# mlcolab/Pathfinder.jl

Measured on AMD Instinct MI355X. Metric: ELBO draws/sec (multipathfinder hot path: fit + ELBO + pool + PSIS + resample), higher is better.
Workload: dtype f64

## Files before the change

### pathfinder.jl_amd/csrc/elbo_kernels.hip

```cpp
#include "pfmi_common.h"
#include "elbo_args.h"
#include "logpdf_lane.h"
#include <stdlib.h>

#define ELBO_THREADS 256


template <int TGT, int RPAD>
struct TargetAcc {
    double q = 0.0, tau = 0.0;
    double tr[RPAD > 0 ? RPAD : 1];
    __device__ __forceinline__ void init() {
#pragma unroll
        for (int j = 0; j < (RPAD > 0 ? RPAD : 1); ++j) tr[j] = 0.0;
    }
    __device__ __forceinline__ void row(const ElboArgs &A, int i, double x) {
        if (TGT == 1) {
            const double e = x - A.t_mean[i];
            q += A.t_a[i] * e * e;
            if (RPAD > 0) {
                const double *wr = A.t_wd + (size_t)i * RPAD;
#pragma unroll
                for (int j = 0; j < RPAD; ++j) tr[j] += wr[j] * e;
            }
        } else if (TGT == 2) {
            if (i == 0) tau = x; else q += x * x;
        }
    }
    __device__ __forceinline__ double finish(const ElboArgs &A) {
        if (TGT == 1) {
            double corr = 0.0;
            if (RPAD > 0) {
#pragma unroll
                for (int j = 0; j < RPAD; ++j) {
                    double g = 0.0;
#pragma unroll
                    for (int l = 0; l <= j; ++l) g += A.t_g[j * RPAD + l] * tr[l];
                    corr += g * g;
// ... 121 lines not shown
#pragma unroll
                for (int j = 0; j < KPAD; ++j) v -= row[j] * tv[j];
                const double xi = mu[i] + sqa[i] * v;
                tg.row(A, i, xi);
                if (X) X[i] = xi;
            }
        }
    }
    *out_lq = ((double)d * PF_LOG2PI + A.logdet[p] + usq) / -2.0;
    *out_lp = tg.finish(A);
}

__global__ __launch_bounds__(256) void pf_elbo_reduce_kernel(int64_t N, const int64_t *__restrict__ off,
                                                             const int32_t *__restrict__ path_of,
                                                             const int32_t *__restrict__ status,
                                                             const double *__restrict__ logp,
                                                             const double *__restrict__ logq,
                                                             double *__restrict__ elbo, double *__restrict__ se,
                                                             int64_t vcap, int seg_len, const int32_t *__restrict__ npts) {
    int p = blockIdx.x;
    const int tid = threadIdx.x;
    if (seg_len > 0) {
        const int k = blockIdx.x / seg_len, l = blockIdx.x - k * seg_len;
        if (l >= npts[k]) return;
        p = (int)((int64_t)k * vcap + l);
    }
    __shared__ double red[8];
    const bool first = ((int64_t)p == off[path_of[p]]);
    if (first || status[p] != PFMI_FIT_OK || N <= 0) {
        if (tid == 0) { elbo[p] = NAN; se[p] = NAN; }
        return;
    }
    const double *lp = logp + (size_t)p * N, *lq = logq + (size_t)p * N;
    double s = 0.0;
    for (int64_t n = tid; n < N; n += 256) s += lp[n] - lq[n];
    s = pf_block_sum1(s, red);
    const double mean = s / (double)N;
    double v = 0.0;
    for (int64_t n = tid; n < N; n += 256) { const double r = (lp[n] - lq[n]) - mean; v += r * r; }
    v = pf_block_sum1(v, red);
    if (tid == 0) {
        elbo[p] = mean;
        se[p] = sqrt((v / (double)(N - 1)) / (double)N);
    }
}

__global__ __launch_bounds__(64) void pf_elbo_argmax_kernel(int K, const int64_t *__restrict__ off, const int32_t *__restrict__ npts,
                                                           const double *__restrict__ elbo, int64_t *__restrict__ best_iter) {
    const int k = blockIdx.x, lane = threadIdx.x;
    if (k >= K) return;
    const int64_t p0 = off[k];
    const int L = npts ? npts[k] - 1 : (int)(off[k + 1] - p0 - 1);
    if (L <= 0) { if (lane == 0) best_iter[k] = 0; return; }
    double xmax = 0.0;
    int imax = 0x7FFFFFFF, have = 0;
    for (int l = 1 + lane; l <= L; l += 64) {
        const double xi = elbo[p0 + l];
        if (isnan(xi)) continue;
        if (!have || xi > xmax) { xmax = xi; imax = l; have = 1; }
    }
#pragma unroll
    for (int o = 32; o >= 1; o >>= 1) {
        const double xo = __shfl_xor(xmax, o, 64);
        const int io = __shfl_xor(imax, o, 64), ho = __shfl_xor(have, o, 64);
        const bool take = ho && (!have || xo > xmax || (xo == xmax && io < imax));
        if (take) { xmax = xo; imax = io; have = 1; }
    }
    if (lane == 0) best_iter[k] = have ? imax : 1;
}

__global__ void pf_logratio_kernel(int64_t n, const double *__restrict__ lp, const double *__restrict__ lq,
                                   double *__restrict__ lr) {
// ... 206 lines not shown
```

### pathfinder.jl_amd/csrc/pfmi_common.h

```cpp
#pragma once
#include <hip/hip_runtime.h>
#include <stdint.h>
#include <chrono>
#include <functional>
#include <memory>
#include <string>
#include <map>
#include <set>
#include <type_traits>
#include <vector>

#include "../../include/pfmi.h"
#include "pfmi_icdftab.h"

#define PF_LOG2PI 1.8378770664093454835606594728112352797227949472755668

void pf_set_error(const char *fmt, ...);
#define PF_HIP(call)                                                                              \
    do {                                                                                          \
        hipError_t e__ = (call);                                                                  \
        if (e__ != hipSuccess) {                                                                  \
            pf_set_error("%s failed: %s (%s:%d)", #call, hipGetErrorString(e__), __FILE__, __LINE__); \
            return PFMI_ERR_HIP;                                                                  \
        }                                                                                         \
// ... 186 lines not shown
    int64_t N_e = 0;
    DevBuf seeds;
    DevBuf logp, logq;
    DevBuf elbo, se;
    DevBuf best_iter;
    DevBuf fit_list;
    DevBuf ubuf;
    DevBuf xbuf;
    DevBuf scratch;
    DevBuf mix;
    DevBuf qf_share_s[2];
    uint32_t qf_epoch_s[2] = {0, 0};
    int qf_slot = 0;
    bool qf_no_share = false;
    int64_t qf_lost_total = 0;
    std::map<std::string, int64_t> qf_plans;
    std::map<std::string, int64_t> draw_plans;
    std::map<std::string, int64_t> fit_plans;

    bool pooled = false;
    int64_t N_r = 0;
    DevBuf pool;
    DevBuf pool_lr;
    DevBuf pool_lp, pool_lq;
    DevBuf pool_points;
    DevBuf pool_seeds;
    int64_t S_w = 0;
    DevBuf lw;
    DevBuf w;
    DevBuf psis_out;
    DevBuf psis_aux;
    DevBuf tailbuf;
    DevBuf cdf;
    DevBuf idx;
    DevBuf gbuf;
    DevBuf sortk, sorti;
    DevBuf cb_x[2], cb_lp[2];
    void *pin_x[2] = {nullptr, nullptr}, *pin_lp[2] = {nullptr, nullptr};
    size_t pin_x_cap = 0, pin_lp_cap = 0;
    hipEvent_t cb_ev[2] = {nullptr, nullptr};
#define PF_DCB_NB 2
    DevBuf dcb_x[PF_DCB_NB], dcb_lp[PF_DCB_NB];
    hipStream_t s_cb[PF_DCB_NB - 1] = {};
    hipEvent_t sg_cb[PF_DCB_NB] = {};
    double cb_seconds = 0.0;
    double cb_bytes_d2h = 0.0;
    double cb_bytes_dev = 0.0;
    bool opt_pending = false;
    LbcState lbc;
    DevBuf lc_X, lc_out, lc_x, lc_g, lc_p, lc_gram, lc_st, lc_ctr;
    int64_t *lc_status = nullptr;
    int32_t opt_K = 0, opt_cap = 0;
    HmcState hmc;
    DevBuf hm_X, hm_out, hm_x0, hm_x, hm_wg, hm_wt, hm_v, hm_st, hm_pts, hm_seeds, hm_eps;
    DevBuf hm_draws, hm_lp, hm_acc, hm_de, hm_div;
    DevBuf hm_pX, hm_pout, hm_pv;
    DevBuf hm_adapt;
    DevBuf hm_scale;
    DevBuf hm_chees;
    DevBuf hm_metric;
    std::vector<double> scale_staged;
    int32_t scale_staged_K = 0;
    DevBuf nt_vec, nt_st, nt_depth, nt_nleap, nt_pev, nt_ctr;
    int64_t *nt_status = nullptr;
    std::map<std::string, int64_t> hmc_plans;
    DevBuf cd_ws, cd_in;
// ... 533 lines not shown
```

### pathfinder.jl_amd/csrc/psis_kernels.hip

```cpp
#include "pfmi_common.h"
#include <stdlib.h>
#include <stddef.h>

#define PSIS_THREADS 1024
#ifndef PSIS_PROF
#define PSIS_PROF 0
#endif
#if PSIS_PROF
#define PS_STAMP(k) do { if (threadIdx.x == 0) { const long long t_ = wall_clock64(); ps_t[k] = t_ - ps_last; ps_last = t_; } } while (0)
#else
#define PS_STAMP(k) do { } while (0)
#endif
#define TAILCAP 4096

#define PF_KEY_NAN 0xFFF8000000000000ull
__device__ __forceinline__ uint64_t pf_key_of(double x) {
    uint64_t b = (uint64_t)__double_as_longlong(x);
    const uint64_t k = (b >> 63) ? ~b : (b | 0x8000000000000000ull);
    return (x != x) ? PF_KEY_NAN : k;
}
__device__ __forceinline__ double pf_val_of(uint64_t k) {
    uint64_t b = (k >> 63) ? (k & 0x7FFFFFFFFFFFFFFFull) : ~k;
    return __longlong_as_double((long long)b);
}
// ... 103 lines not shown
    const unsigned long long ti = st->prefix;
    int npow = 1;
    while (npow < R) npow <<= 1;
    for (int t = tid; t < npow; t += nt) { tkeys[t] = ~0ull; tidx[t] = 0xFFFFFFFFu; }
    if (tid == 0) st->count = 0u;
    __syncthreads();
    pf_foreach_batched(vals, S, [&](long long i, double x) {
        const uint64_t k = pf_key_of(x);
        if (k > tk || (k == tk && (unsigned long long)i >= ti)) {
            const unsigned slot = atomicAdd(&st->count, 1u);
            if (slot < (unsigned)TAILCAP) { tkeys[slot] = k; tidx[slot] = (uint32_t)i; }
        }
    });
    __syncthreads();
    for (int size = 2; size <= npow; size <<= 1) {
        for (int stride = size >> 1; stride > 0; stride >>= 1) {
            for (int t = tid; t < npow / 2; t += nt) {
                const int lo = 2 * t - (t & (stride - 1));
                const int hi = lo + stride;
                const bool up = ((lo & size) == 0);
                const uint64_t ka = tkeys[lo], kb = tkeys[hi];
                const uint32_t ia = tidx[lo], ib = tidx[hi];
                const bool a_gt_b = (ka > kb) || (ka == kb && ia > ib);
                if (a_gt_b == up) { tkeys[lo] = kb; tkeys[hi] = ka; tidx[lo] = ib; tidx[hi] = ia; }
            }
            __syncthreads();
        }
    }
}

#define PSIS_MULTI_MIN 8192
#define PSIS_MW 64
#define PSIS_MT 256
struct PsisAux {
    unsigned long long kmax, kmin_inv;
    unsigned hist[4096];
    unsigned cand_count, done, replaced, ti0;
    unsigned long long tk0;
    double mx, se_tail, pareto_k, sigma;
    int M, pad;
    double partial[PSIS_MW];
    unsigned long long cand_key[TAILCAP];
    unsigned cand_idx[TAILCAP];
    double tail_val[TAILCAP];
    unsigned tail_idx[TAILCAP];
};
__device__ __forceinline__ int pf_psis_shift0(unsigned long long kmin, unsigned long long kmax) {
    const unsigned long long diff = kmin ^ kmax;
    const int top = diff ? 63 - __clzll((long long)diff) : 0;
    return top >= 11 ? top - 11 : 0;
}
__global__ __launch_bounds__(PSIS_MT) void pf_psis_minmax_kernel(long long S, const double *__restrict__ lr, PsisAux *aux) {
    unsigned long long kmax = 0ull, kinv = 0ull;
    for (long long i = (long long)blockIdx.x * PSIS_MT + threadIdx.x; i < S; i += (long long)PSIS_MW * PSIS_MT) {
        const unsigned long long k = pf_key_of(lr[i]);
        kmax = k > kmax ? k : kmax; kinv = ~k > kinv ? ~k : kinv;
    }
    for (int off = 32; off > 0; off >>= 1) {
        const unsigned long long a = __shfl_xor(kmax, off, 64), b = __shfl_xor(kinv, off, 64);
        kmax = a > kmax ? a : kmax; kinv = b > kinv ? b : kinv;
    }
    if ((threadIdx.x & 63) == 0) { atomicMax(&aux->kmax, kmax); atomicMax(&aux->kmin_inv, kinv); }
}
__global__ __launch_bounds__(PSIS_MT) void pf_psis_hist_kernel(long long S, const double *__restrict__ lr, PsisAux *aux) {
    __shared__ unsigned h[4096];
    for (int b = threadIdx.x; b < 4096; b += PSIS_MT) h[b] = 0u;
    __syncthreads();
    const int sh = pf_psis_shift0(~aux->kmin_inv, aux->kmax);
    for (long long i = (long long)blockIdx.x * PSIS_MT + threadIdx.x; i < S; i += (long long)PSIS_MW * PSIS_MT)
        atomicAdd(&h[(unsigned)((pf_key_of(lr[i]) >> sh) & 0xFFFull)], 1u);
    __syncthreads();
    for (int b = threadIdx.x; b < 4096; b += PSIS_MT) if (h[b]) atomicAdd(&aux->hist[b], h[b]);
}
__global__ __launch_bounds__(PSIS_MT) void pf_psis_compact_kernel(long long S, const double *__restrict__ lr, PsisAux *aux, int R) {
    __shared__ unsigned part[PSIS_MT];
    __shared__ int s_bin, s_ok;
    const int tid = threadIdx.x;
    unsigned loc[16], sum = 0u;
#pragma unroll
// ... 9 lines not shown
            if (cum < (unsigned)R && cum + loc[j] >= (unsigned)R) { s_bin = 4095 - 16 * tid - j; s_ok = (cum + loc[j] <= (unsigned)TAILCAP); break; }
            cum += loc[j];
        }
    }
    __syncthreads();
    const int bin = s_bin;
    if (blockIdx.x == 0 && tid == 0) aux->done = (bin >= 0 && s_ok) ? 1u : 0u;
    if (bin < 0 || !s_ok) return;
    const int sh = pf_psis_shift0(~aux->kmin_inv, aux->kmax);
    for (long long i = (long long)blockIdx.x * PSIS_MT + tid; i < S; i += (long long)PSIS_MW * PSIS_MT) {
        const unsigned long long k = pf_key_of(lr[i]);
        if ((int)((k >> sh) & 0xFFFull) >= bin) {
            const unsigned slot = atomicAdd(&aux->cand_count, 1u);
            if (slot < (unsigned)TAILCAP) { aux->cand_key[slot] = k; aux->cand_idx[slot] = (unsigned)i; }
        }
    }
}
__device__ __forceinline__ bool pf_psis_is_tail(const PsisAux *aux, long long i, double x) {
    const unsigned long long k = pf_key_of(x);
    return aux->replaced && (k > aux->tk0 || (k == aux->tk0 && (unsigned long long)i > (unsigned long long)aux->ti0));
}
__global__ __launch_bounds__(PSIS_MT) void pf_psis_sum_kernel(long long S, const double *__restrict__ lr, PsisAux *aux) {
    __shared__ double red[PSIS_MT / 64];
    const double mx = aux->mx;
    double se = 0.0;
    if (isfinite(mx))
        for (long long i = (long long)blockIdx.x * PSIS_MT + threadIdx.x; i < S; i += (long long)PSIS_MW * PSIS_MT) {
            const double x = lr[i];
            if (!pf_psis_is_tail(aux, i, x)) se += exp(x - mx);
        }
    se = pf_block_sum1(se, red);
    if (threadIdx.x == 0) aux->partial[blockIdx.x] = se;
}
__global__ __launch_bounds__(PSIS_MT) void pf_psis_norm_kernel(long long S, const double *__restrict__ lr, const PsisAux *aux,
                                                              double *__restrict__ lw, double *__restrict__ wout,
                                                              double *__restrict__ out, const double *__restrict__ tail_val,
                                                              const unsigned *__restrict__ tail_idx) {
    if (tail_val == nullptr) { tail_val = aux->tail_val; tail_idx = aux->tail_idx; }
    const double mx = aux->mx;
    double se = aux->se_tail;
    for (int b = 0; b < PSIS_MW; ++b) se += aux->partial[b];
    const double lse = isfinite(mx) ? mx + log(se) : mx;
    for (long long i = (long long)blockIdx.x * PSIS_MT + threadIdx.x; i < S; i += (long long)PSIS_MW * PSIS_MT) {
        const double x = lr[i];
        if (!pf_psis_is_tail(aux, i, x)) { const double v = x - lse; lw[i] = v; wout[i] = exp(v); }
    }
    if (blockIdx.x == 0) {
        if (aux->replaced)
            for (int t = threadIdx.x; t < aux->M; t += PSIS_MT) {
                const double v = tail_val[t] - lse;
                lw[tail_idx[t]] = v; wout[tail_idx[t]] = exp(v);
            }
        if (threadIdx.x == 0) { out[0] = aux->pareto_k; out[1] = (double)aux->M; out[2] = aux->sigma; out[3] = lse; }
    }
}

template <bool MULTI>
__device__ __forceinline__ void pf_psis_segment(long long S, const double *__restrict__ lr, double *__restrict__ lw,
                                                double *__restrict__ wout, double *__restrict__ out, int M, PsisAux *aux) {
    const int tid = threadIdx.x, nt = blockDim.x, lane = tid & 63, wave = tid >> 6, nw = nt >> 6;
    __shared__ uint64_t tkeys[TAILCAP];
    __shared__ uint32_t tidx[TAILCAP];
    __shared__ SelectState st;
    __shared__ double red[PSIS_THREADS / 64];
    __shared__ double s_theta[128], s_ll[128];
    __shared__ double s_sigma, s_mu;

#if PSIS_PROF
    long long ps_t[8] = {0, 0, 0, 0, 0, 0, 0, 0}, ps_last = wall_clock64();
#endif
    double pareto_k = NAN;
    bool have_sel = false, replaced = false;
    uint64_t tk0 = 0; uint32_t ti0 = 0; double lmax_all = NAN, logu_all = NAN;
    if (tid == 0) s_sigma = NAN;
    __syncthreads();
    if (M >= 5 && M + 1 <= TAILCAP && (long long)(M + 1) <= S) {
        if (MULTI && aux->done) {
            const int R = M + 1, cnt = (int)aux->cand_count;
            int npow = 1;
            while (npow < cnt) npow <<= 1;
            for (int t = tid; t < npow; t += nt) {
                tkeys[t] = t < cnt ? aux->cand_key[t] : ~0ull;
                tidx[t] = t < cnt ? aux->cand_idx[t] : 0xFFFFFFFFu;
            }
            __syncthreads();
            for (int size = 2; size <= npow; size <<= 1)
                for (int stride = size >> 1; stride > 0; stride >>= 1) {
                    for (int t = tid; t < npow / 2; t += nt) {
                        const int lo = 2 * t - (t & (stride - 1)), hi = lo + stride;
                        const bool up = ((lo & size) == 0);
                        const uint64_t ka = tkeys[lo], kb = tkeys[hi];
                        const uint32_t ia = tidx[lo], ib = tidx[hi];
                        const bool a_gt_b = (ka > kb) || (ka == kb && ia > ib);
                        if (a_gt_b == up) { tkeys[lo] = kb; tkeys[hi] = ka; tidx[lo] = ib; tidx[hi] = ia; }
                    }
                    __syncthreads();
                }
            uint64_t mk[(TAILCAP + PSIS_THREADS - 1) / PSIS_THREADS];
            uint32_t mi[(TAILCAP + PSIS_THREADS - 1) / PSIS_THREADS];
#pragma unroll
            for (int q = 0; q < (TAILCAP + PSIS_THREADS - 1) / PSIS_THREADS; ++q) {
                const int t = tid + q * nt;
                if (t < R) { mk[q] = tkeys[cnt - R + t]; mi[q] = tidx[cnt - R + t]; }
            }
            __syncthreads();
// ... 5 lines not shown
            __syncthreads();
        } else pf_select_top_sorted(lr, S, M + 1, tkeys, tidx, &st);
        PS_STAMP(0);
        double *w = reinterpret_cast<double *>(tkeys);
        const double logu = pf_val_of(tkeys[0]);
        const double lmax = pf_val_of(tkeys[M]);
        have_sel = true; tk0 = tkeys[0]; ti0 = tidx[0]; lmax_all = lmax; logu_all = logu;
        double bad = 0.0;
        for (int t = 1 + tid; t <= M; t += nt) if (!isfinite(pf_val_of(tkeys[t]))) bad = 1.0;
        bad = pf_block_sum1(bad, red);
        __syncthreads();
        if (bad == 0.0) {
            const double mu_s = exp(logu - lmax);
            double vals[(TAILCAP + PSIS_THREADS - 1) / PSIS_THREADS];
            double nz = 0.0;
#pragma unroll
            for (int q = 0; q < (TAILCAP + PSIS_THREADS - 1) / PSIS_THREADS; ++q) {
                const int t = tid + q * nt;
                vals[q] = (t < M) ? (exp(pf_val_of(tkeys[t + 1]) - lmax) - mu_s) : 0.0;
                if (t < M && vals[q] != 0.0) nz = 1.0;
            }
            nz = pf_block_sum1(nz, red);
            __syncthreads();
#pragma unroll
            for (int q = 0; q < (TAILCAP + PSIS_THREADS - 1) / PSIS_THREADS; ++q) {
                const int t = tid + q * nt;
                if (t < M) w[t] = vals[q];
            }
            __syncthreads();
            PS_STAMP(1);
            if (nz > 0.0) {
                const int mest = 30 + (int)floor(sqrt((double)M));
                const double xstar = w[(M + 2) / 4 - 1], xmax = w[M - 1];
                for (int i = wave; i < mest; i += nw) {
                    const double p = ((double)(i + 1) - 0.5) / (double)mest;
                    const double theta = 1.0 / xmax + (1.0 - sqrt(1.0 / p)) / (3.0 * xstar);
                    double kk = 0.0;
                    for (int t = lane; t < M; t += 64) kk += log1p(-theta * w[t]);
                    kk = pf_wave_sum(kk) / (double)M;
                    if (lane == 0) {
                        s_theta[i] = theta;
                        s_ll[i] = (double)M * (log(-theta / kk) - kk - 1.0);
                    }
                }
                __syncthreads();
                PS_STAMP(2);
                if (tid < 64) {
                    double lmx = -INFINITY;
                    for (int i = lane; i < mest; i += 64) lmx = fmax(lmx, s_ll[i]);
                    lmx = pf_wave_max(lmx);
                    double ws = 0.0, ts = 0.0;
                    for (int i = lane; i < mest; i += 64) { const double e = exp(s_ll[i] - lmx); ws += e; ts += e * s_theta[i]; }
                    ws = pf_wave_sum(ws); ts = pf_wave_sum(ts);
                    if (lane == 0) s_mu = ts / ws;
                }
                __syncthreads();
                const double th = s_mu;
                double kk = 0.0;
                for (int t = tid; t < M; t += nt) kk += log1p(-th * w[t]);
                kk = pf_block_sum1(kk, red) / (double)M;
                const double sigma = -kk / th;
                double kadj = kk;
                if (isfinite(kk)) kadj = (kk * (double)M + 5.0) / ((double)M + 10.0);
                pareto_k = kadj;
                PS_STAMP(3);
                if (isfinite(kadj) && isfinite(sigma)) {
                    __syncthreads();
                    for (int t = tid; t < M; t += nt) {
                        const double p = ((double)(t + 1) - 0.5) / (double)M;
                        const double nl = -log1p(-p);
                        const double z = (kadj == 0.0) ? nl : expm1(kadj * nl) / kadj;
                        double v = log(sigma * z + mu_s);
                        if (v > 0.0) v = 0.0;
                        w[t] = v + lmax;
                    }
                    replaced = true;
                }
                if (tid == 0) s_sigma = sigma;
            }
        }
    }
    __threadfence_block();
    __syncthreads();
    PS_STAMP(4);
    const double *wt = reinterpret_cast<const double *>(tkeys);
    auto is_tail = [&](long long i, double x) {
        const uint64_t k = pf_key_of(x);
        return replaced && (k > tk0 || (k == tk0 && (uint64_t)i > (uint64_t)ti0));
    };
    double mx = -INFINITY;
    if (replaced) {
        for (int t = tid; t < M; t += nt) mx = fmax(mx, wt[t]);
        mx = fmax(pf_block_max1(mx, red), logu_all);
    } else if (have_sel) mx = lmax_all;
    else {
        pf_foreach_batched(lr, S, [&](long long, double x) { mx = fmax(mx, x); });
        mx = pf_block_max1(mx, red);
    }
    __syncthreads();
    if (MULTI) {
        double se = 0.0;
        if (replaced && isfinite(mx)) for (int t = tid; t < M; t += nt) se += exp(wt[t] - mx);
        se = pf_block_sum1(se, red);
        if (replaced) for (int t = tid; t < M; t += nt) { aux->tail_val[t] = wt[t]; aux->tail_idx[t] = tidx[t + 1]; }
        if (tid == 0) {
            aux->mx = mx; aux->se_tail = se; aux->replaced = replaced ? 1u : 0u; aux->tk0 = tk0; aux->ti0 = ti0;
            aux->pareto_k = pareto_k; aux->sigma = s_sigma; aux->M = M;
        }
#if PSIS_PROF
        PS_STAMP(5);
        if (tid == 0) printf("PSIS_PROF multi S %lld M %d (10 ns): select+sort %lld vals %lld grid %lld mean+k %lld smooth %lld hand-over %lld\n", S, M, ps_t[0], ps_t[1], ps_t[2], ps_t[3], ps_t[4], ps_t[5]);
#endif
        return;
    }
// ... 29 lines not shown
    pf_psis_segment<MULTI>(S, lr, lw, wout, out, M, aux);
}

__global__ __launch_bounds__(PSIS_THREADS) void pf_psis_runs_kernel(long long N_r, const double *__restrict__ lr, double *__restrict__ lw,
                                                                    double *__restrict__ wout, double *__restrict__ out5, int M) {
    __shared__ double red[PSIS_THREADS / 64];
    const size_t base = (size_t)blockIdx.x * (size_t)N_r;
    double *o = out5 + (size_t)blockIdx.x * PF_PSIS_RUN_OUT;
    pf_psis_segment<false>(N_r, lr + base, lw + base, wout + base, o, M, nullptr);
    __syncthreads();
    const double *w = wout + base;
    double ss = 0.0;
    for (long long i = threadIdx.x; i < N_r; i += PSIS_THREADS) { const double x = w[i]; ss += x * x; }
    ss = pf_block_sum1(ss, red);
    if (threadIdx.x == 0) o[4] = ss;
}

__device__ __forceinline__ uint64_t pf_weight_to_fixed(double w) {
    if (!(w > 0.0)) return 0ull;
    if (w >= 1.0) return 1ull << 62;
    return (uint64_t)floor(w * 4611686018427387904.0);
}
__device__ __forceinline__ uint64_t pf_uniform_to_bits(double u) {
    return ((uint64_t)floor(u * 9007199254740992.0)) << 11;
}
__device__ __forceinline__ uint64_t pf_wave_scan_u64(uint64_t v, int lane) {
#pragma unroll
    for (int off = 1; off < 64; off <<= 1) {
        const unsigned lo = __shfl_up((unsigned)v, off, 64), hi = __shfl_up((unsigned)(v >> 32), off, 64);
        if (lane >= off) v += ((uint64_t)hi << 32) | lo;
    }
    return v;
}
__global__ __launch_bounds__(PSIS_THREADS) void pf_cdf_kernel(long long S, const double *__restrict__ w,
                                                              uint64_t *__restrict__ cdf) {
    const int tid = threadIdx.x, lane = tid & 63, wave = tid >> 6, nw = blockDim.x >> 6;
    __shared__ uint64_t part[PSIS_THREADS / 64];
    const long long ntile = (S + 255) >> 8, per = (ntile + nw - 1) / nw;
    const long long t0 = (long long)wave * per, t1 = (t0 + per < ntile) ? t0 + per : ntile;
    auto load4 = [&](const long long t, uint64_t (&x)[4]) {
        const long long i = (t << 8) + 4 * lane;
        if (i + 3 < S) {
#pragma unroll
            for (int e = 0; e < 4; ++e) x[e] = pf_weight_to_fixed(w[i + e]);
        } else {
#pragma unroll
            for (int e = 0; e < 4; ++e) x[e] = (i + e < S) ? pf_weight_to_fixed(w[i + e]) : 0ull;
        }
    };
    uint64_t s = 0;
    for (long long t = t0; t < t1; ++t) {
        uint64_t x[4];
        load4(t, x);
        s += (x[0] + x[1]) + (x[2] + x[3]);
    }
    s = pf_wave_scan_u64(s, lane);
    if (lane == 63) part[wave] = s;
    __syncthreads();
    uint64_t carry = 0;
    for (int v = 0; v < wave; ++v) carry += part[v];
    for (long long t = t0; t < t1; ++t) {
        uint64_t x[4];
        load4(t, x);
        x[1] += x[0]; x[2] += x[1]; x[3] += x[2];
        const uint64_t incl = pf_wave_scan_u64(x[3], lane);
        const uint64_t base = carry + (incl - x[3]);
        const long long i = (t << 8) + 4 * lane;
#pragma unroll
        for (int e = 0; e < 4; ++e) if (i + e < S) cdf[i + e] = base + x[e];
        carry += ((uint64_t)__shfl((unsigned)(incl >> 32), 63, 64) << 32) | (uint64_t)__shfl((unsigned)incl, 63, 64);
    }
}
__global__ void pf_sample_kernel(long long S, long long ndraws, int weighted, uint64_t seed,
                                 const double *__restrict__ uniforms, const uint64_t *__restrict__ cdf,
                                 int64_t *__restrict__ idx, int *__restrict__ err) {
    const long long t = (long long)blockIdx.x * blockDim.x + threadIdx.x;
    if (t >= ndraws) return;
    const uint64_t R = uniforms ? pf_uniform_to_bits(uniforms[t]) : pf_rand_u64(seed, (uint64_t)t, 1u);
    if (!weighted) { idx[t] = (int64_t)__umul64hi(R, (uint64_t)S); return; }
    const uint64_t Q = cdf[S - 1];
    if (Q == 0) { if (t == 0) *err = 1; idx[t] = 0; return; }
    const uint64_t r = __umul64hi(R, Q);
    long long lo = 0, hi = S - 1;
    while (lo < hi) { const long long mid = (lo + hi) >> 1; if (cdf[mid] > r) hi = mid; else lo = mid + 1; }
    idx[t] = lo;
}

__global__ void pf_norep_keys_kernel(long long S, int weighted, uint64_t seed, const double *__restrict__ w,
                                     double *__restrict__ negkey) {
    const long long i = (long long)blockIdx.x * blockDim.x + threadIdx.x;
    if (i >= S) return;
    const uint64_t R = pf_rand_u64(seed, (uint64_t)i, 2u);
    const double u = ((double)(R >> 11) + 0.5) * 1.1102230246251565404e-16;
    const double wi = weighted ? w[i] : 1.0;
    negkey[i] = (wi > 0.0) ? -(-log(u) / wi) : -INFINITY;
}
__global__ __launch_bounds__(PSIS_THREADS) void pf_norep_select_kernel(long long S, int ndraws,
                                                                       const double *__restrict__ negkey,
                                                                       int64_t *__restrict__ idx, int *__restrict__ err) {
    __shared__ uint64_t tkeys[TAILCAP];
    __shared__ uint32_t tidx[TAILCAP];
    __shared__ SelectState st;
    pf_select_top_sorted(negkey, S, ndraws, tkeys, tidx, &st);
    for (int t = threadIdx.x; t < ndraws; t += blockDim.x) {
        idx[t] = (int64_t)tidx[ndraws - 1 - t];
        if (!isfinite(pf_val_of(tkeys[ndraws - 1 - t]))) *err = 1;
    }
}

__global__ void pf_sortkeys_init_kernel(long long S, long long n2, const double *__restrict__ negkey, uint64_t *__restrict__ keys,
                                        uint32_t *__restrict__ ids) {
    const long long i = (long long)blockIdx.x * blockDim.x + threadIdx.x;
    if (i >= n2) return;
    keys[i] = (i < S) ? pf_key_of(-negkey[i]) : ~0ull;
    ids[i] = (uint32_t)i;
}
__global__ void pf_bitonic_step_kernel(long long n2, long long j, long long k, uint64_t *__restrict__ keys, uint32_t *__restrict__ ids) {
    const long long i = (long long)blockIdx.x * blockDim.x + threadIdx.x;
    if (i >= n2) return;
    const long long l = i ^ j;
    if (l <= i) return;
    const uint64_t ka = keys[i], kb = keys[l];
    const uint32_t ia = ids[i], ib = ids[l];
    const bool a_gt_b = (ka > kb) || (ka == kb && ia > ib);
// ... 154 lines not shown
                    double v = log(sigma * z + mu_s);
                    if (v > 0.0) v = 0.0;
                    w[t] = v + lmax;
                }
                replaced = true;
            }
            if (tid == 0) s_sigma = sigma;
        }
    }
    __threadfence_block();
    __syncthreads();
    double mx = lmax;
    if (replaced) {
        mx = -INFINITY;
        for (int t = tid; t < M; t += nt) mx = fmax(mx, w[t]);
        mx = fmax(pf_block_max1(mx, red), logu);
    }
    __syncthreads();
    double se = 0.0;
    if (replaced && isfinite(mx)) for (int t = tid; t < M; t += nt) se += exp(w[t] - mx);
    se = pf_block_sum1(se, red);
    if (tid == 0) {
        aux->mx = mx; aux->se_tail = se; aux->replaced = replaced ? 1u : 0u; aux->tk0 = tkeys[0]; aux->ti0 = tidx[0];
        aux->pareto_k = pareto_k; aux->sigma = s_sigma; aux->M = M;
    }
}

static long long psis_tail_length(long long S) {
    long long a = (S + 4) / 5;
    long long b = (long long)ceil(3.0 * sqrt((double)S));
    return a < b ? a : b;
}

int32_t pf_launch_psis(pfmi_ctx *c, const double *d_lr, int64_t S) {
    PF_CHECK(S > 0, PFMI_ERR_ARG, "psis: empty log-ratio vector");
    PF_CHECK(S < (1ll << 32), PFMI_ERR_UNSUPPORTED, "psis: S too large");
    const long long M = psis_tail_length(S);
    PF_TRY(c->lw.ensure(sizeof(double) * S));
    PF_TRY(c->w.ensure(sizeof(double) * S));
    PF_TRY(c->psis_out.ensure(sizeof(double) * 4));
    pf_kernel_begin(c);
    const char *force = pf_debug_get("PFMI_PSIS_KERNEL");
    if (M + 1 > TAILCAP || (force && force[0] == 'b' && M >= 5 && M + 1 <= S)) {
        long long n2 = 1;
        while (n2 < S) n2 <<= 1;
        PF_TRY(c->sortk.ensure(sizeof(uint64_t) * (size_t)n2));
        PF_TRY(c->sorti.ensure(sizeof(uint32_t) * (size_t)n2));
        PF_TRY(c->psis_aux.ensure(sizeof(PsisAux)));
        PF_TRY(c->scratch.ensure(sizeof(double) * (size_t)(M + 1)));
        PsisAux *aux = c->psis_aux.as<PsisAux>();
        PF_HIP(hipMemsetAsync(aux, 0, offsetof(PsisAux, cand_key), c->stream));
        const dim3 grid((unsigned)((n2 + 255) / 256));
        hipLaunchKernelGGL(pf_sortkeys_init_lr_kernel, grid, dim3(256), 0, c->stream, (long long)S, n2, d_lr, c->sortk.as<uint64_t>(),
                           c->sorti.as<uint32_t>());
        for (long long k = 2; k <= n2; k <<= 1)
            for (long long j = k >> 1; j > 0; j >>= 1)
                hipLaunchKernelGGL(pf_bitonic_step_kernel, grid, dim3(256), 0, c->stream, n2, j, k, c->sortk.as<uint64_t>(),
                                   c->sorti.as<uint32_t>());
        const uint64_t *tk = c->sortk.as<uint64_t>() + (n2 - (M + 1));
        const uint32_t *ti = c->sorti.as<uint32_t>() + (n2 - (M + 1));
        hipLaunchKernelGGL(pf_psis_bigtail_kernel, dim3(1), dim3(PSIS_THREADS), 0, c->stream, (int)M, tk, ti, c->scratch.as<double>(), aux);
        hipLaunchKernelGGL(pf_psis_sum_kernel, dim3(PSIS_MW), dim3(PSIS_MT), 0, c->stream, (long long)S, d_lr, aux);
        hipLaunchKernelGGL(pf_psis_norm_kernel, dim3(PSIS_MW), dim3(PSIS_MT), 0, c->stream, (long long)S, d_lr, aux,
                           c->lw.as<double>(), c->w.as<double>(), c->psis_out.as<double>(), (const double *)c->scratch.as<double>(),
                           (const unsigned *)(ti + 1));
    } else if (S >= PSIS_MULTI_MIN && M >= 5 && !(force && force[0] == 's')) {
        PF_TRY(c->psis_aux.ensure(sizeof(PsisAux)));
        PsisAux *aux = c->psis_aux.as<PsisAux>();
        PF_HIP(hipMemsetAsync(aux, 0, offsetof(PsisAux, cand_key), c->stream));
        hipLaunchKernelGGL(pf_psis_minmax_kernel, dim3(PSIS_MW), dim3(PSIS_MT), 0, c->stream, (long long)S, d_lr, aux);
        hipLaunchKernelGGL(pf_psis_hist_kernel, dim3(PSIS_MW), dim3(PSIS_MT), 0, c->stream, (long long)S, d_lr, aux);
        hipLaunchKernelGGL(pf_psis_compact_kernel, dim3(PSIS_MW), dim3(PSIS_MT), 0, c->stream, (long long)S, d_lr, aux, (int)M + 1);
        hipLaunchKernelGGL(pf_psis_kernel<true>, dim3(1), dim3(PSIS_THREADS), 0, c->stream, (long long)S, d_lr,
                           c->lw.as<double>(), c->w.as<double>(), c->psis_out.as<double>(), (int)M, aux);
        hipLaunchKernelGGL(pf_psis_sum_kernel, dim3(PSIS_MW), dim3(PSIS_MT), 0, c->stream, (long long)S, d_lr, aux);
        hipLaunchKernelGGL(pf_psis_norm_kernel, dim3(PSIS_MW), dim3(PSIS_MT), 0, c->stream, (long long)S, d_lr, aux,
                           c->lw.as<double>(), c->w.as<double>(), c->psis_out.as<double>(), (const double *)nullptr, (const unsigned *)nullptr);
    } else
        hipLaunchKernelGGL(pf_psis_kernel<false>, dim3(1), dim3(PSIS_THREADS), 0, c->stream, (long long)S, d_lr,
                           c->lw.as<double>(), c->w.as<double>(), c->psis_out.as<double>(), (int)M, (PsisAux *)nullptr);
    pf_kernel_end(c, "psis");
    PF_HIP(hipGetLastError());
    c->S_w = S;
    return PFMI_OK;
}

int32_t pf_launch_psis_runs(pfmi_ctx *c, const double *d_lr, int K, int64_t N_r) {
    PF_CHECK(K >= 1 && N_r >= 1, PFMI_ERR_ARG, "psis_runs: empty pool");
    const long long M = psis_tail_length(N_r);
    PF_CHECK(M + 1 <= TAILCAP, PFMI_ERR_UNSUPPORTED, "psis_runs: %lld draws per run need a tail of %lld, beyond the one-workgroup route (%d)",
             (long long)N_r, M, TAILCAP - 1);
    const size_t S = (size_t)K * (size_t)N_r;
    PF_TRY(c->runs_lw.ensure(sizeof(double) * S));
    PF_TRY(c->runs_w.ensure(sizeof(double) * S));
    PF_TRY(c->runs_out.ensure(sizeof(double) * PF_PSIS_RUN_OUT * (size_t)K));
    pf_kernel_begin(c);
    hipLaunchKernelGGL(pf_psis_runs_kernel, dim3((unsigned)K), dim3(PSIS_THREADS), 0, c->stream, (long long)N_r, d_lr, c->runs_lw.as<double>(),
                       c->runs_w.as<double>(), c->runs_out.as<double>(), (int)M);
    pf_kernel_end(c, "psis_runs");
    PF_HIP(hipGetLastError());
    return PFMI_OK;
}

int32_t pf_enqueue_resample(pfmi_ctx *c, int64_t S, int64_t ndraws, int importance, int replace, uint64_t seed,
                            const double *d_uniforms) {
    PF_TRY(c->idx.ensure(sizeof(int64_t) * (ndraws > 0 ? ndraws : 1)));
    PF_TRY(c->scratch.ensure(sizeof(double) * (S > 0 ? S : 1) + 64));
    PF_TRY(c->rs_err.ensure(sizeof(int)));
    int *d_err = c->rs_err.as<int>();
    PF_HIP(hipMemsetAsync(d_err, 0, sizeof(int), c->stream));
    pf_kernel_begin(c);
    if (replace) {
        if (importance) {
            PF_TRY(c->cdf.ensure(sizeof(uint64_t) * S));
            hipLaunchKernelGGL(pf_cdf_kernel, dim3(1), dim3(PSIS_THREADS), 0, c->stream, (long long)S,
                               c->w.as<double>(), c->cdf.as<uint64_t>());
        }
        hipLaunchKernelGGL(pf_sample_kernel, dim3((unsigned)((ndraws + 255) / 256)), dim3(256), 0, c->stream,
                           (long long)S, (long long)ndraws, importance, seed, d_uniforms, c->cdf.as<uint64_t>(),
                           c->idx.as<int64_t>(), d_err);
    } else {
        PF_CHECK(ndraws <= S, PFMI_ERR_ARG, "cannot draw %lld without replacement from %lld", (long long)ndraws,
                 (long long)S);
        hipLaunchKernelGGL(pf_norep_keys_kernel, dim3((unsigned)((S + 255) / 256)), dim3(256), 0, c->stream,
                           (long long)S, importance, seed, c->w.as<double>(), c->scratch.as<double>());
        if (ndraws <= TAILCAP) {
            hipLaunchKernelGGL(pf_norep_select_kernel, dim3(1), dim3(PSIS_THREADS), 0, c->stream, (long long)S,
                               (int)ndraws, c->scratch.as<double>(), c->idx.as<int64_t>(), d_err);
        } else {
            long long n2 = 1;
            while (n2 < S) n2 <<= 1;
            PF_TRY(c->sortk.ensure(sizeof(uint64_t) * (size_t)n2));
            PF_TRY(c->sorti.ensure(sizeof(uint32_t) * (size_t)n2));
            const dim3 grid((unsigned)((n2 + 255) / 256));
            hipLaunchKernelGGL(pf_sortkeys_init_kernel, grid, dim3(256), 0, c->stream, (long long)S, n2, c->scratch.as<double>(),
                               c->sortk.as<uint64_t>(), c->sorti.as<uint32_t>());
            for (long long k = 2; k <= n2; k <<= 1)
                for (long long j = k >> 1; j > 0; j >>= 1)
                    hipLaunchKernelGGL(pf_bitonic_step_kernel, grid, dim3(256), 0, c->stream, n2, j, k, c->sortk.as<uint64_t>(),
                                       c->sorti.as<uint32_t>());
            hipLaunchKernelGGL(pf_sorted_take_kernel, dim3((unsigned)((ndraws + 255) / 256)), dim3(256), 0, c->stream,
                               (long long)ndraws, c->sortk.as<uint64_t>(), c->sorti.as<uint32_t>(), c->idx.as<int64_t>(), d_err);
        }
    }
    pf_kernel_end(c, "resample");
    PF_HIP(hipGetLastError());
    return PFMI_OK;
}

int32_t pf_resample_check(pfmi_ctx *c) {
    int err = 0;
    PF_TRY(pf_download(c, &err, c->rs_err.p, sizeof(int)));
    PF_TRY(pf_stream_sync(c));
    PF_CHECK(err == 0, PFMI_ERR_NUMERIC, "resample: weights are all zero / not enough positive weights");
    return PFMI_OK;
}

int32_t pf_launch_resample(pfmi_ctx *c, int64_t S, int64_t ndraws, int importance, int replace, uint64_t seed,
// ... 49 lines not shown
```

Measured before the change: 531.4 million.

## Parallelize CDF scan and PSIS k-hat grid across workgroups; cache ELBO residuals

The importance-resampling CDF moves from a single-workgroup scan to a multi-block tiled scan that uses a last-arriver ticket, and sampling does a two-level binary search over tile totals and then within the tile. The PSIS Pareto k-hat grid evaluation is spread across 16 workgroups, with the last arriver collecting the results. PSIS aux and resample error resets now happen inside kernels instead of through per-call memsets. The ELBO reduction keeps log-ratios in registers for small N so the second pass does not reload them. The atomic ticket and self-reset schemes add cross-block state that must stay consistent between calls.

```diff
diff --git a/pathfinder.jl_amd/csrc/elbo_kernels.hip b/pathfinder.jl_amd/csrc/elbo_kernels.hip
--- a/pathfinder.jl_amd/csrc/elbo_kernels.hip
+++ b/pathfinder.jl_amd/csrc/elbo_kernels.hip
@@ -4,6 +4,7 @@
 #include <stdlib.h>
 
 #define ELBO_THREADS 256
+#define ELBO_RED_KEEP 8
 
 
 template <int TGT, int RPAD>
@@ -191,12 +192,26 @@
         return;
     }
     const double *lp = logp + (size_t)p * N, *lq = logq + (size_t)p * N;
-    double s = 0.0;
-    for (int64_t n = tid; n < N; n += 256) s += lp[n] - lq[n];
-    s = pf_block_sum1(s, red);
-    const double mean = s / (double)N;
-    double v = 0.0;
-    for (int64_t n = tid; n < N; n += 256) { const double r = (lp[n] - lq[n]) - mean; v += r * r; }
+    double s = 0.0, v = 0.0, mean;
+    if (N <= 256 * ELBO_RED_KEEP) {
+        double lr[ELBO_RED_KEEP];
+#pragma unroll
+        for (int u = 0; u < ELBO_RED_KEEP; ++u) {
+            const int64_t n = tid + 256 * u;
+            lr[u] = n < N ? lp[n] - lq[n] : 0.0;
+        }
+#pragma unroll
+        for (int u = 0; u < ELBO_RED_KEEP; ++u) if (tid + 256 * u < N) s += lr[u];
+        s = pf_block_sum1(s, red);
+        mean = s / (double)N;
+#pragma unroll
+        for (int u = 0; u < ELBO_RED_KEEP; ++u) if (tid + 256 * u < N) { const double r = lr[u] - mean; v += r * r; }
+    } else {
+        for (int64_t n = tid; n < N; n += 256) s += lp[n] - lq[n];
+        s = pf_block_sum1(s, red);
+        mean = s / (double)N;
+        for (int64_t n = tid; n < N; n += 256) { const double r = (lp[n] - lq[n]) - mean; v += r * r; }
+    }
     v = pf_block_sum1(v, red);
     if (tid == 0) {
         elbo[p] = mean;
diff --git a/pathfinder.jl_amd/csrc/pfmi_common.h b/pathfinder.jl_amd/csrc/pfmi_common.h
--- a/pathfinder.jl_amd/csrc/pfmi_common.h
+++ b/pathfinder.jl_amd/csrc/pfmi_common.h
@@ -242,6 +242,7 @@
     DevBuf psis_aux;
     DevBuf tailbuf;
     DevBuf cdf;
+    unsigned *cdf_ticket = nullptr;
     DevBuf idx;
     DevBuf gbuf;
     DevBuf sortk, sorti;
diff --git a/pathfinder.jl_amd/csrc/psis_kernels.hip b/pathfinder.jl_amd/csrc/psis_kernels.hip
--- a/pathfinder.jl_amd/csrc/psis_kernels.hip
+++ b/pathfinder.jl_amd/csrc/psis_kernels.hip
@@ -159,19 +159,36 @@
 #define PSIS_MULTI_MIN 8192
 #define PSIS_MW 64
 #define PSIS_MT 256
+#define PSIS_FW 16
 struct PsisAux {
     unsigned long long kmax, kmin_inv;
     unsigned hist[4096];
     unsigned cand_count, done, replaced, ti0;
+    unsigned ticket, pad0;
     unsigned long long tk0;
     double mx, se_tail, pareto_k, sigma;
     int M, pad;
     double partial[PSIS_MW];
+    double g_theta[128], g_ll[128];
     unsigned long long cand_key[TAILCAP];
     unsigned cand_idx[TAILCAP];
     double tail_val[TAILCAP];
     unsigned tail_idx[TAILCAP];
 };
+__device__ __forceinline__ bool pf_last_arriver(unsigned *ticket, int *s_last) {
+    __threadfence();
+    __syncthreads();
+    if (threadIdx.x == 0) {
+        const unsigned n = gridDim.x * gridDim.y;
+        const int last = atomicAdd(ticket, 1u) == n - 1u;
+        if (last) *ticket = 0u;
+        *s_last = last;
+    }
+    __syncthreads();
+    const bool last = *s_last != 0;
+    if (last) __threadfence();
+    return last;
+}
 __device__ __forceinline__ int pf_psis_shift0(unsigned long long kmin, unsigned long long kmax) {
     const unsigned long long diff = kmin ^ kmax;
     const int top = diff ? 63 - __clzll((long long)diff) : 0;
@@ -247,7 +264,7 @@
     se = pf_block_sum1(se, red);
     if (threadIdx.x == 0) aux->partial[blockIdx.x] = se;
 }
-__global__ __launch_bounds__(PSIS_MT) void pf_psis_norm_kernel(long long S, const double *__restrict__ lr, const PsisAux *aux,
+__global__ __launch_bounds__(PSIS_MT) void pf_psis_norm_kernel(long long S, const double *__restrict__ lr, PsisAux *aux,
                                                               double *__restrict__ lw, double *__restrict__ wout,
                                                               double *__restrict__ out, const double *__restrict__ tail_val,
                                                               const unsigned *__restrict__ tail_idx) {
@@ -268,6 +285,10 @@
             }
         if (threadIdx.x == 0) { out[0] = aux->pareto_k; out[1] = (double)aux->M; out[2] = aux->sigma; out[3] = lse; }
     }
+    if (blockIdx.x == PSIS_MW - 1) {
+        for (int b = threadIdx.x; b < 4096; b += PSIS_MT) aux->hist[b] = 0u;
+        if (threadIdx.x == 0) { aux->kmax = 0ull; aux->kmin_inv = 0ull; aux->cand_count = 0u; }
+    }
 }
 
 template <bool MULTI>
@@ -286,6 +307,7 @@
 #endif
     double pareto_k = NAN;
     bool have_sel = false, replaced = false;
+    bool past_grid = false;
     uint64_t tk0 = 0; uint32_t ti0 = 0; double lmax_all = NAN, logu_all = NAN;
     if (tid == 0) s_sigma = NAN;
     __syncthreads();
@@ -357,16 +379,25 @@
             if (nz > 0.0) {
                 const int mest = 30 + (int)floor(sqrt((double)M));
                 const double xstar = w[(M + 2) / 4 - 1], xmax = w[M - 1];
-                for (int i = wave; i < mest; i += nw) {
+                const int g0 = MULTI ? (int)blockIdx.x * nw : 0, gstep = MULTI ? nw * (int)gridDim.x : nw;
+                for (int i = g0 + wave; i < mest; i += gstep) {
                     const double p = ((double)(i + 1) - 0.5) / (double)mest;
                     const double theta = 1.0 / xmax + (1.0 - sqrt(1.0 / p)) / (3.0 * xstar);
                     double kk = 0.0;
                     for (int t = lane; t < M; t += 64) kk += log1p(-theta * w[t]);
                     kk = pf_wave_sum(kk) / (double)M;
                     if (lane == 0) {
+                        const double ll = (double)M * (log(-theta / kk) - kk - 1.0);
                         s_theta[i] = theta;
-                        s_ll[i] = (double)M * (log(-theta / kk) - kk - 1.0);
+                        s_ll[i] = ll;
+                        if (MULTI) { aux->g_theta[i] = theta; aux->g_ll[i] = ll; }
                     }
+                }
+                if (MULTI) {
+                    __shared__ int s_last;
+                    if (!pf_last_arriver(&aux->ticket, &s_last)) return;
+                    for (int i = tid; i < mest; i += nt) { s_theta[i] = aux->g_theta[i]; s_ll[i] = aux->g_ll[i]; }
+                    past_grid = true;
                 }
                 __syncthreads();
                 PS_STAMP(2);
@@ -405,6 +436,7 @@
             }
         }
     }
+    if (MULTI && !past_grid && blockIdx.x != 0) return;
     __threadfence_block();
     __syncthreads();
     PS_STAMP(4);
@@ -500,64 +532,63 @@
     }
     return v;
 }
-__global__ __launch_bounds__(PSIS_THREADS) void pf_cdf_kernel(long long S, const double *__restrict__ w,
-                                                              uint64_t *__restrict__ cdf) {
-    const int tid = threadIdx.x, lane = tid & 63, wave = tid >> 6, nw = blockDim.x >> 6;
-    __shared__ uint64_t part[PSIS_THREADS / 64];
-    const long long ntile = (S + 255) >> 8, per = (ntile + nw - 1) / nw;
-    const long long t0 = (long long)wave * per, t1 = (t0 + per < ntile) ? t0 + per : ntile;
-    auto load4 = [&](const long long t, uint64_t (&x)[4]) {
+#define CDF_THREADS 256
+__global__ __launch_bounds__(CDF_THREADS) void pf_cdf_kernel(long long S, const double *__restrict__ w, uint64_t *__restrict__ cdf,
+                                                            uint64_t *tile, unsigned *ticket) {
+    const int tid = threadIdx.x, lane = tid & 63, wave = tid >> 6;
+    __shared__ uint64_t part[CDF_THREADS / 64];
+    __shared__ int s_last;
+    const long long ntile = (S + 255) >> 8;
+    const long long t = (long long)blockIdx.x * (CDF_THREADS / 64) + wave;
+    if (t < ntile) {
         const long long i = (t << 8) + 4 * lane;
-        if (i + 3 < S) {
-#pragma unroll
-            for (int e = 0; e < 4; ++e) x[e] = pf_weight_to_fixed(w[i + e]);
-        } else {
-#pragma unroll
-            for (int e = 0; e < 4; ++e) x[e] = (i + e < S) ? pf_weight_to_fixed(w[i + e]) : 0ull;
-        }
-    };
-    uint64_t s = 0;
-    for (long long t = t0; t < t1; ++t) {
         uint64_t x[4];
-        load4(t, x);
-        s += (x[0] + x[1]) + (x[2] + x[3]);
-    }
-    s = pf_wave_scan_u64(s, lane);
-    if (lane == 63) part[wave] = s;
-    __syncthreads();
-    uint64_t carry = 0;
-    for (int v = 0; v < wave; ++v) carry += part[v];
-    for (long long t = t0; t < t1; ++t) {
-        uint64_t x[4];
-        load4(t, x);
+#pragma unroll
+        for (int e = 0; e < 4; ++e) x[e] = (i + e < S) ? pf_weight_to_fixed(w[i + e]) : 0ull;
         x[1] += x[0]; x[2] += x[1]; x[3] += x[2];
         const uint64_t incl = pf_wave_scan_u64(x[3], lane);
-        const uint64_t base = carry + (incl - x[3]);
-        const long long i = (t << 8) + 4 * lane;
+        const uint64_t base = incl - x[3];
 #pragma unroll
         for (int e = 0; e < 4; ++e) if (i + e < S) cdf[i + e] = base + x[e];
-        carry += ((uint64_t)__shfl((unsigned)(incl >> 32), 63, 64) << 32) | (uint64_t)__shfl((unsigned)incl, 63, 64);
-    }
+        if (lane == 63) tile[t] = incl;
+    }
+    if (!pf_last_arriver(ticket, &s_last)) return;
+    const long long per = (ntile + CDF_THREADS - 1) / CDF_THREADS;
+    const long long a = ((long long)tid * per < ntile) ? (long long)tid * per : ntile, b = (a + per < ntile) ? a + per : ntile;
+    uint64_t s = 0;
+    for (long long j = a; j < b; ++j) s += tile[j];
+    const uint64_t incl = pf_wave_scan_u64(s, lane);
+    if (lane == 63) part[wave] = incl;
+    __syncthreads();
+    uint64_t carry = incl - s;
+    for (int v = 0; v < wave; ++v) carry += part[v];
+    for (long long j = a; j < b; ++j) { carry += tile[j]; tile[j] = carry; }
 }
 __global__ void pf_sample_kernel(long long S, long long ndraws, int weighted, uint64_t seed,
                                  const double *__restrict__ uniforms, const uint64_t *__restrict__ cdf,
-                                 int64_t *__restrict__ idx, int *__restrict__ err) {
+                                 const uint64_t *__restrict__ tile, int64_t *__restrict__ idx, int *__restrict__ err) {
     const long long t = (long long)blockIdx.x * blockDim.x + threadIdx.x;
     if (t >= ndraws) return;
     const uint64_t R = uniforms ? pf_uniform_to_bits(uniforms[t]) : pf_rand_u64(seed, (uint64_t)t, 1u);
-    if (!weighted) { idx[t] = (int64_t)__umul64hi(R, (uint64_t)S); return; }
-    const uint64_t Q = cdf[S - 1];
-    if (Q == 0) { if (t == 0) *err = 1; idx[t] = 0; return; }
+    if (!weighted) { if (t == 0) *err = 0; idx[t] = (int64_t)__umul64hi(R, (uint64_t)S); return; }
+    const long long ntile = (S + 255) >> 8;
+    const uint64_t Q = tile[ntile - 1];
+    if (t == 0) *err = (Q == 0) ? 1 : 0;
+    if (Q == 0) { idx[t] = 0; return; }
     const uint64_t r = __umul64hi(R, Q);
-    long long lo = 0, hi = S - 1;
-    while (lo < hi) { const long long mid = (lo + hi) >> 1; if (cdf[mid] > r) hi = mid; else lo = mid + 1; }
-    idx[t] = lo;
+    long long lo = 0, hi = ntile - 1;
+    while (lo < hi) { const long long mid = (lo + hi) >> 1; if (tile[mid] > r) hi = mid; else lo = mid + 1; }
+    const uint64_t rr = r - (lo ? tile[lo - 1] : 0ull);
+    long long a = lo << 8, b = ((a + 256 < S) ? a + 256 : S) - 1;
+    while (a < b) { const long long mid = (a + b) >> 1; if (cdf[mid] > rr) b = mid; else a = mid + 1; }
+    idx[t] = a;
 }
 
 __global__ void pf_norep_keys_kernel(long long S, int weighted, uint64_t seed, const double *__restrict__ w,
-                                     double *__restrict__ negkey) {
+                                     double *__restrict__ negkey, int *__restrict__ err) {
     const long long i = (long long)blockIdx.x * blockDim.x + threadIdx.x;
     if (i >= S) return;
+    if (i == 0) *err = 0;
     const uint64_t R = pf_rand_u64(seed, (uint64_t)i, 2u);
     const double u = ((double)(R >> 11) + 0.5) * 1.1102230246251565404e-16;
     const double wi = weighted ? w[i] : 1.0;
@@ -778,6 +809,13 @@
     return a < b ? a : b;
 }
 
+static int32_t psis_aux_ensure(pfmi_ctx *c) {
+    if (c->psis_aux.cap >= sizeof(PsisAux)) return PFMI_OK;
+    PF_TRY(c->psis_aux.ensure(sizeof(PsisAux)));
+    PF_HIP(hipMemsetAsync(c->psis_aux.p, 0, offsetof(PsisAux, cand_key), c->stream));
+    return PFMI_OK;
+}
+
 int32_t pf_launch_psis(pfmi_ctx *c, const double *d_lr, int64_t S) {
     PF_CHECK(S > 0, PFMI_ERR_ARG, "psis: empty log-ratio vector");
     PF_CHECK(S < (1ll << 32), PFMI_ERR_UNSUPPORTED, "psis: S too large");
@@ -792,10 +830,9 @@
         while (n2 < S) n2 <<= 1;
         PF_TRY(c->sortk.ensure(sizeof(uint64_t) * (size_t)n2));
         PF_TRY(c->sorti.ensure(sizeof(uint32_t) * (size_t)n2));
-        PF_TRY(c->psis_aux.ensure(sizeof(PsisAux)));
+        PF_TRY(psis_aux_ensure(c));
         PF_TRY(c->scratch.ensure(sizeof(double) * (size_t)(M + 1)));
         PsisAux *aux = c->psis_aux.as<PsisAux>();
-        PF_HIP(hipMemsetAsync(aux, 0, offsetof(PsisAux, cand_key), c->stream));
         const dim3 grid((unsigned)((n2 + 255) / 256));
         hipLaunchKernelGGL(pf_sortkeys_init_lr_kernel, grid, dim3(256), 0, c->stream, (long long)S, n2, d_lr, c->sortk.as<uint64_t>(),
                            c->sorti.as<uint32_t>());
@@ -811,13 +848,12 @@
                            c->lw.as<double>(), c->w.as<double>(), c->psis_out.as<double>(), (const double *)c->scratch.as<double>(),
                            (const unsigned *)(ti + 1));
     } else if (S >= PSIS_MULTI_MIN && M >= 5 && !(force && force[0] == 's')) {
-        PF_TRY(c->psis_aux.ensure(sizeof(PsisAux)));
+        PF_TRY(psis_aux_ensure(c));
         PsisAux *aux = c->psis_aux.as<PsisAux>();
-        PF_HIP(hipMemsetAsync(aux, 0, offsetof(PsisAux, cand_key), c->stream));
         hipLaunchKernelGGL(pf_psis_minmax_kernel, dim3(PSIS_MW), dim3(PSIS_MT), 0, c->stream, (long long)S, d_lr, aux);
         hipLaunchKernelGGL(pf_psis_hist_kernel, dim3(PSIS_MW), dim3(PSIS_MT), 0, c->stream, (long long)S, d_lr, aux);
         hipLaunchKernelGGL(pf_psis_compact_kernel, dim3(PSIS_MW), dim3(PSIS_MT), 0, c->stream, (long long)S, d_lr, aux, (int)M + 1);
-        hipLaunchKernelGGL(pf_psis_kernel<true>, dim3(1), dim3(PSIS_THREADS), 0, c->stream, (long long)S, d_lr,
+        hipLaunchKernelGGL(pf_psis_kernel<true>, dim3(PSIS_FW), dim3(PSIS_THREADS), 0, c->stream, (long long)S, d_lr,
                            c->lw.as<double>(), c->w.as<double>(), c->psis_out.as<double>(), (int)M, aux);
         hipLaunchKernelGGL(pf_psis_sum_kernel, dim3(PSIS_MW), dim3(PSIS_MT), 0, c->stream, (long long)S, d_lr, aux);
         hipLaunchKernelGGL(pf_psis_norm_kernel, dim3(PSIS_MW), dim3(PSIS_MT), 0, c->stream, (long long)S, d_lr, aux,
@@ -854,22 +890,30 @@
     PF_TRY(c->scratch.ensure(sizeof(double) * (S > 0 ? S : 1) + 64));
     PF_TRY(c->rs_err.ensure(sizeof(int)));
     int *d_err = c->rs_err.as<int>();
-    PF_HIP(hipMemsetAsync(d_err, 0, sizeof(int), c->stream));
+    if (ndraws <= 0) PF_HIP(hipMemsetAsync(d_err, 0, sizeof(int), c->stream));
     pf_kernel_begin(c);
     if (replace) {
+        const long long ntile = ((long long)S + 255) >> 8;
+        uint64_t *d_tile = nullptr;
         if (importance) {
-            PF_TRY(c->cdf.ensure(sizeof(uint64_t) * S));
-            hipLaunchKernelGGL(pf_cdf_kernel, dim3(1), dim3(PSIS_THREADS), 0, c->stream, (long long)S,
-                               c->w.as<double>(), c->cdf.as<uint64_t>());
+            const size_t need = sizeof(uint64_t) * ((size_t)S + (size_t)ntile + 1);
+            if (c->cdf.cap < need) {
+                PF_TRY(c->cdf.ensure(need));
+                c->cdf_ticket = reinterpret_cast<unsigned *>(c->cdf.as<char>() + c->cdf.cap - sizeof(uint64_t));
+                PF_HIP(hipMemsetAsync(c->cdf_ticket, 0, sizeof(uint64_t), c->stream));
+            }
+            d_tile = c->cdf.as<uint64_t>() + S;
+            hipLaunchKernelGGL(pf_cdf_kernel, dim3((unsigned)((ntile + CDF_THREADS / 64 - 1) / (CDF_THREADS / 64))), dim3(CDF_THREADS), 0, c->stream,
+                               (long long)S, c->w.as<double>(), c->cdf.as<uint64_t>(), d_tile, c->cdf_ticket);
         }
         hipLaunchKernelGGL(pf_sample_kernel, dim3((unsigned)((ndraws + 255) / 256)), dim3(256), 0, c->stream,
                            (long long)S, (long long)ndraws, importance, seed, d_uniforms, c->cdf.as<uint64_t>(),
-                           c->idx.as<int64_t>(), d_err);
+                           (const uint64_t *)d_tile, c->idx.as<int64_t>(), d_err);
     } else {
         PF_CHECK(ndraws <= S, PFMI_ERR_ARG, "cannot draw %lld without replacement from %lld", (long long)ndraws,
                  (long long)S);
         hipLaunchKernelGGL(pf_norep_keys_kernel, dim3((unsigned)((S + 255) / 256)), dim3(256), 0, c->stream,
-                           (long long)S, importance, seed, c->w.as<double>(), c->scratch.as<double>());
+                           (long long)S, importance, seed, c->w.as<double>(), c->scratch.as<double>(), d_err);
         if (ndraws <= TAILCAP) {
             hipLaunchKernelGGL(pf_norep_select_kernel, dim3(1), dim3(PSIS_THREADS), 0, c->stream, (long long)S,
                                (int)ndraws, c->scratch.as<double>(), c->idx.as<int64_t>(), d_err);
```

Measured after the change: 533.7 million, median of 6. No clear change (+0.4%).
